# seanbonjean/llm-sharding

Measured on AMD Instinct MI355X. Metric: output_tokens_per_sec_whole_node, higher is better.
Workload: dtype bf16; 1 GPU; model=Llama-2-7B, global_batch=512, seq_len=303, parallelism=pp1, microbatches=1, batch_per_microbatch=512, prompt_len=128, concurrent_streams=1, max_seq=320

## Files before the change

csrc/build.py:

```python
#!/usr/bin/env python3
from __future__ import annotations

import argparse
import concurrent.futures as cf
import glob
import os
import shutil
import subprocess
import sys

ROOT = os.path.dirname(os.path.dirname(os.path.abspath(__file__)))
CSRC = os.path.join(ROOT, "csrc")
OUT = os.path.join(ROOT, "llm_sharding_amd", "_native")
OBJ = os.path.join(ROOT, "build", "obj")
ROCM = os.environ.get("ROCM_PATH", "/opt/rocm")


def _hipcc() -> str:
    p = os.path.join(ROCM, "bin", "hipcc")
    return p if os.path.exists(p) else (shutil.which("hipcc") or "hipcc")


def _newest_header() -> float:
    hs = glob.glob(os.path.join(CSRC, "**", "*.h"), recursive=True)
    return max((os.path.getmtime(h) for h in hs), default=0.0)


def _stale(src: str, obj: str, hdr_mtime: float) -> bool:
    if not os.path.exists(obj):
        return True
    t = os.path.getmtime(obj)
    return t < os.path.getmtime(src) or t < hdr_mtime


def _run(cmd: list) -> None:
    r = subprocess.run(cmd, stdout=subprocess.PIPE, stderr=subprocess.STDOUT, text=True)
    if r.returncode != 0:
        raise RuntimeError(f"build failed: {' '.join(cmd)}\n{r.stdout}")
    if r.stdout.strip():
        sys.stderr.write(r.stdout)


def build(force: bool = False, jobs: int = 8, arch: str = "gfx950", verbose: bool = True) -> dict:
    os.makedirs(OUT, exist_ok=True)
    os.makedirs(OBJ, exist_ok=True)
    hdr = _newest_header()
    hipcc = _hipcc()
    kernel_srcs = sorted(glob.glob(os.path.join(CSRC, "kernels", "*.hip")) +
                         glob.glob(os.path.join(CSRC, "sampling", "*.hip")) +
                         glob.glob(os.path.join(CSRC, "cache", "*.hip")) +
                         glob.glob(os.path.join(CSRC, "spec", "*.hip")) +
                         glob.glob(os.path.join(CSRC, "quant", "*.hip")))
    comm_srcs = sorted(glob.glob(os.path.join(CSRC, "comm", "*.cpp")))
    hip_flags = ["-O3", "-std=c++17", "-fPIC", f"--offload-arch={arch}", "-Wall",
                 "-Wno-unused-function", "-munsafe-fp-atomics", "-fno-slp-vectorize"]
    stamp = os.path.join(OBJ, "hip_flags.txt")
    if (open(stamp).read() if os.path.exists(stamp) else "") != " ".join(hip_flags):
        force = True
    jobs_list = []
    kobjs = []
    for s in kernel_srcs:
        o = os.path.join(OBJ, os.path.basename(s) + ".o")
        kobjs.append(o)
        if force or _stale(s, o, hdr):
            jobs_list.append([hipcc, *hip_flags, "-c", s, "-o", o])
    cobjs = []
    cxx = shutil.which("g++") or "g++"
    for s in comm_srcs:
        o = os.path.join(OBJ, os.path.basename(s) + ".o")
        cobjs.append(o)
        if force or _stale(s, o, hdr):
            jobs_list.append([cxx, "-O2", "-std=c++17", "-fPIC", "-Wall", "-c", s, "-o", o])
    if verbose and jobs_list:
        print(f"[build] compiling {len(jobs_list)} translation unit(s) for {arch}", file=sys.stderr)
    with cf.ThreadPoolExecutor(max(1, jobs)) as ex:
        list(ex.map(_run, jobs_list))
    out = {}
    klib = os.path.join(OUT, "liblsa_kernels.so")
    manifest = os.path.join(OBJ, "liblsa_kernels.objs")
    listed = open(manifest).read() if os.path.exists(manifest) else ""
    if kobjs and (force or not os.path.exists(klib) or listed != "\n".join(kobjs) or
                  os.path.getmtime(klib) < max(os.path.getmtime(o) for o in kobjs)):
        _run([hipcc, "-shared", "-fPIC", f"--offload-arch={arch}", *kobjs, "-o", klib])
        with open(manifest, "w") as f:
            f.write("\n".join(kobjs))
    with open(stamp, "w") as f:
        f.write(" ".join(hip_flags))
    audit_stamp = os.path.join(OBJ, "isa_audit.ok")
    if not os.path.exists(audit_stamp) or os.path.getmtime(audit_stamp) < os.path.getmtime(klib):
        sys.path.insert(0, CSRC)
        from isa_audit import audit
        res = audit(klib, arch)
        if res["code_objects"] == 0:
            raise RuntimeError(f"ISA audit of {klib}: no {arch} code object found in the library's offload bundle")
        if res["findings"]:
            raise RuntimeError(f"ISA audit of {klib}: back-to-back hazards {res['by_rule']}, e.g. "
                               f"{res['findings'][:3]} (csrc/isa_audit.py)")
        with open(audit_stamp, "w") as f:
            f.write(f"{res['code_objects']} code objects, {res['packed_fp32_instructions']} packed FP32 (explicit "
                    f"vector code), 0 findings under rules {sorted(res['by_rule'])}\n")
    out["kernels"] = klib
    clib = os.path.join(OUT, "liblsa_comm.so")
    if cobjs and (force or not os.path.exists(clib) or
                  os.path.getmtime(clib) < max(os.path.getmtime(o) for o in cobjs)):
        _run([cxx, "-shared", "-fPIC", *cobjs, "-o", clib, "-lpthread"])
    out["comm"] = clib
    return out


def main() -> None:
    ap = argparse.ArgumentParser()
    ap.add_argument("--force", action="store_true")
    ap.add_argument("-j", "--jobs", type=int, default=min(8, os.cpu_count() or 4))
    ap.add_argument("--arch", default=os.environ.get("PYTORCH_ROCM_ARCH", "gfx950"))
    a = ap.parse_args()
    res = build(a.force, a.jobs, a.arch)
    for k, v in res.items():
        print(f"{k}: {v}")


if __name__ == "__main__":
    main()
```

llm_sharding_amd/runtime/engine_int4.py:

```python
from __future__ import annotations

from typing import Optional

import torch

from ..ops import int4, packing
from .engine import StageEngine

PROJ = ("qkv", "o", "gate_up", "down")


class Int4StageEngine(StageEngine):
    def __init__(self, cfg, start: int, end: int, device="cpu", dtype=torch.bfloat16, *, weight_dtype: str = "int4",
                 **kw):
        if weight_dtype != "int4":
            raise ValueError(f"Int4StageEngine holds int4 weights, got weight_dtype={weight_dtype!r}")
        self.int4 = torch.device(device).type == "cuda"
        if self.int4:
            for name, (n, k) in zip(PROJ, self.proj_shapes(cfg)):
                if k % int4.INT4_GROUP:
                    raise ValueError(f"weight_dtype='int4' needs K % {int4.INT4_GROUP} == 0: the {name} projection "
                                     f"has K={k}")
        super().__init__(cfg, start, end, device, dtype, weight_dtype="bf16", **kw)

    def _prepare_layer(self, lw: dict):
        out = super()._prepare_layer(lw)
        if not self.int4:
            return out
        for name in PROJ:
            q, sc = int4.quantize_int4_groups(packing.unpack_b(getattr(out, name)))
            setattr(out, name, int4.pack_b_int4(q))
            setattr(out, name + "_s", int4.pack_scales_int4(sc))
        return out

    def _alloc_runtime(self) -> None:
        super()._alloc_runtime()
        if self.int4:
            shapes = self.proj_shapes(self.cfg)
            self.w_scratch = torch.empty(max(n * k for n, k in shapes), dtype=torch.bfloat16, device=self.device)

    def _forward_hip(self, h, slot, pos, kv_len, rows, nsplit: Optional[int] = None, tiles=None) -> torch.Tensor:
        from ..ops import hip
        cfg = self.cfg
        H, I, eps = cfg.hidden_size, cfg.intermediate_size, cfg.rms_norm_eps
        nh, nkv, hd = cfg.num_attention_heads, cfg.num_key_value_heads, cfg.head_dim
        if rows > self.max_prefill_rows and rows > self.DECODE_MAX_ROWS:
            raise ValueError(f"{rows} rows exceed max_prefill_rows={self.max_prefill_rows}")
        if h.dtype != torch.bfloat16 or not h.is_contiguous():
            h = h.to(torch.bfloat16).contiguous()
        hbuf = self.buf_h[:rows]
        if h.data_ptr() != hbuf.data_ptr():
            hbuf.copy_(h)
        decode = rows <= self.DECODE_MAX_ROWS
        if nsplit is None and tiles is None:
            kv_max = self.max_seq if decode else (int(pos.max().item()) + 1 if kv_len is None else int(kv_len.max().item()))
            nsplit = self._attn_nsplit(rows, kv_max)
        q, attn_o, act, xn = self.buf_q[:rows], self.buf_attn[:rows], self.buf_act[:rows], self.buf_xn[:rows]
        ws = self.coop_ws
        native_fp8 = False
        native_int4 = rows <= int4.INT4_MAX_ROWS
        if cfg.is_gpt2:
            return self._forward_hip_gpt2(hbuf, slot, pos, kv_len, rows, nsplit, tiles, decode, native_int4)
        wbf = self._weights_bf16

        def dec(x, w, s, N, K, epi, ep, norm=False):
            if native_int4:
                int4.gemv_int4(x, w, s, rows, N, K, epi, ep, norm=norm, eps=eps)
            else:
                hip.gemv(x, wbf(w, s, N, K), rows, N, K, epi, ep, norm=norm, eps=eps, ws=ws)

        def dec_resid(x, w, s, N, K, ep):
            pc = None if (native_fp8 or s is not None or cfg.is_gpt2 or N not in (2048, 4096, 6144, 8192)) \
                else packing.partial_config(N // 16, rows, k=K)
            if pc is None or ws.slab.numel() < pc[3] * rows * N:
                dec(x, w, s, N, K, hip.EPI_RESID, ep)
                return
            part = ws.slab[:pc[3] * rows * N].view(pc[3], rows, N)
            hip.gemv(x, w, rows, N, K, hip.EPI_PARTIAL, hip.make_epi(out=part, ldo=N), coop=pc, ws=ws,
                     out_numel=part.numel())
            hip.resid_rmsnorm_partials(hbuf, part, pc[3], rows, eps)

        def pre(x, w, s, N, K, epi, ep):
            hip.gemm(x, wbf(w, s, N, K), rows, N, K, epi, ep, ws=ws, sk_ws=self.sk_ws)

        proj_gemm = (not decode) or (rows > self.GEMV_MAX_ROWS and not native_fp8 and self.sk_ws is not None)
        part_ok = proj_gemm and self.part_k is not None and rows <= self.part_k.shape[1]

        def resid_proj(x, w, s, N, K, ep):
            pp = hip.gemm_sk_partial_plan(rows, N, K) if part_ok else None
            if pp is None:
                pre(x, w, s, N, K, hip.EPI_RESID, ep)
                return 0
            bn, sp = pp
            hip.gemm_sk(x, wbf(w, s, N, K), rows, N, K, hip.EPI_PARTIAL, hip.make_epi(out=self.part_k, ldo=N),
                        bn=bn, grid=hip.N_CU, dp=0, split=sp, ws=self.sk_ws, out_numel=self.part_k.numel())
            return sp

        fuse = proj_gemm and self.ss_buf is not None and rows <= self.ss_buf.shape[0]
        ss = self.ss_buf[:rows] if fuse else None
        ao = (self.ATTN_OPROJ and rows == 1 and tiles is None and nsplit == 1 and not proj_gemm and not native_fp8
              and self.ao_sync is not None)
        ss_valid = False
        pending = 0
        for li, lw in enumerate(self.layers):
            kc, vc = self.k_cache[li], self.v_cache[li]
            ep_qkv = hip.make_epi(out=q, k_cache=kc, v_cache=vc, slot=slot, pos=pos, cos=self.cos, sin=self.sin,
                                  ldo=q.stride(0), n_heads=nh, n_kv=nkv, head_dim=hd, t_max=self.max_seq)
            if not proj_gemm:
                dec(hbuf, lw.qkv, lw.qkv_s, cfg.qkv_size, H, hip.EPI_QKV, ep_qkv, norm=True)
            else:
                if pending and not fuse:
                    hip.resid_rmsnorm_partials(hbuf, self.part_k, pending, rows, eps, out=xn)
                    pending = 0
                    pre(xn, lw.qkv, lw.qkv_s, cfg.qkv_size, H, hip.EPI_QKV, ep_qkv)
                elif fuse:
                    if pending:
                        hip.resid_rmsnorm_partials(hbuf, self.part_k, pending, rows, eps)
                        pending = 0
                    if not ss_valid:
                        hip.row_ss(hbuf, rows, ss)
                    ep_qkv = hip.make_epi(out=q, k_cache=kc, v_cache=vc, slot=slot, pos=pos, cos=self.cos,
                                          sin=self.sin, ldo=q.stride(0), n_heads=nh, n_kv=nkv, head_dim=hd,
                                          t_max=self.max_seq, ss_in=ss, ss_eps=eps)
                    pre(hbuf, lw.qkv, lw.qkv_s, cfg.qkv_size, H, hip.EPI_QKV, ep_qkv)
                else:
                    hip.rmsnorm(hbuf, None, xn, rows, eps, H)
                    pre(xn, lw.qkv, lw.qkv_s, cfg.qkv_size, H, hip.EPI_QKV, ep_qkv)
            ep_o = hip.make_epi(out=hbuf, resid=hbuf, ldo=hbuf.stride(0), ldr=hbuf.stride(0))
            fused_o = ao and lw.o_s is None and hip.attn_oproj(q, kc, vc, slot, pos, nh, nkv, hd, attn_o, lw.o, H, ep_o,
                                                               self.ao_sync, kv_len=kv_len)
            if tiles is not None:
                hip.attn_prefill(q, kc, vc, tiles[1], nh, nkv, hd, attn_o, causal=kv_len is None, tiles_host=tiles[0])
            elif not fused_o:
                hip.attn(q, kc, vc, slot, pos, rows, nh, nkv, hd, nsplit, self.part_o, self.part_lse, attn_o,
                         kv_len=kv_len, counters=self.attn_cnt, min_chunk=self.ATTN_MIN_CHUNK)
            ep_gu = hip.make_epi(out=act, ldo=act.stride(0))
            if not proj_gemm:
                if not fused_o:
                    dec_resid(attn_o, lw.o, lw.o_s, H, cfg.q_size, ep_o)
                dec(hbuf, lw.gate_up, lw.gate_up_s, 2 * I, H, hip.EPI_SWIGLU, ep_gu, norm=True)
                dec_resid(act, lw.down, lw.down_s, H, I, ep_o)
            else:
                ep_r = hip.make_epi(out=hbuf, resid=hbuf, ldo=hbuf.stride(0), ldr=hbuf.stride(0), ss_out=ss) \
                    if fuse else ep_o
                sp = resid_proj(attn_o, lw.o, lw.o_s, H, cfg.q_size, ep_r)
                if sp:
                    hip.resid_rmsnorm_partials(hbuf, self.part_k, sp, rows, eps, out=xn)
                    pre(xn, lw.gate_up, lw.gate_up_s, 2 * I, H, hip.EPI_SWIGLU, ep_gu)
                elif fuse:
                    pre(hbuf, lw.gate_up, lw.gate_up_s, 2 * I, H, hip.EPI_SWIGLU,
                        hip.make_epi(out=act, ldo=act.stride(0), ss_in=ss, ss_eps=eps))
                else:
                    hip.rmsnorm(hbuf, None, xn, rows, eps, H)
                    pre(xn, lw.gate_up, lw.gate_up_s, 2 * I, H, hip.EPI_SWIGLU, ep_gu)
                pending = resid_proj(act, lw.down, lw.down_s, H, I, ep_r)
                ss_valid = fuse and not pending
        if pending:
            hip.resid_rmsnorm_partials(hbuf, self.part_k, pending, rows, eps)
        return hbuf

    def _weights_bf16(self, w, s, N, K):
        return w if s is None else int4.dequant_int4_packed(w, s, self.w_scratch, N, K)

    def _forward_hip_gpt2(self, hbuf, slot, pos, kv_len, rows, nsplit, tiles, decode, native_int4) -> torch.Tensor:
        from ..ops import hip
        cfg = self.cfg
        H, I, eps = cfg.hidden_size, cfg.intermediate_size, cfg.rms_norm_eps
        nh, nkv, hd = cfg.num_attention_heads, cfg.num_key_value_heads, cfg.head_dim
        q, attn_o, act, xn = self.buf_q[:rows], self.buf_attn[:rows], self.buf_act[:rows], self.buf_xn[:rows]
        ws = self.coop_ws

        def proj(x, w, s, N, K, epi, ep):
            if decode and native_int4:
                int4.gemv_int4(x, w, s, rows, N, K, epi, ep)
                return
            wb = self._weights_bf16(w, s, N, K)
            if decode:
                hip.gemv(x, wb, rows, N, K, epi, ep, ws=ws)
            else:
                hip.gemm(x, wb, rows, N, K, epi, ep, ws=ws, sk_ws=self.sk_ws)

        for li, lw in enumerate(self.layers):
            kc, vc = self.k_cache[li], self.v_cache[li]
            pe = self.pos_emb if (li == 0 and self.start == 0) else None
            hip.layernorm(hbuf, xn, lw.ln_in, lw.ln_in_b, rows, eps, pos_emb=pe, pos=pos)
            ep_qkv = hip.make_epi(out=q, k_cache=kc, v_cache=vc, slot=slot, pos=pos, ldo=q.stride(0), n_heads=nh,
                                  n_kv=nkv, head_dim=hd, t_max=self.max_seq, bias=lw.qkv_b)
            proj(xn, lw.qkv, lw.qkv_s, cfg.qkv_size, H, hip.EPI_QKV, ep_qkv)
            if tiles is not None:
                hip.attn_prefill(q, kc, vc, tiles[1], nh, nkv, hd, attn_o, causal=kv_len is None, tiles_host=tiles[0])
            else:
                hip.attn(q, kc, vc, slot, pos, rows, nh, nkv, hd, nsplit, self.part_o, self.part_lse, attn_o,
                         kv_len=kv_len, counters=self.attn_cnt, min_chunk=self.ATTN_MIN_CHUNK)
            proj(attn_o, lw.o, lw.o_s, H, cfg.q_size, hip.EPI_RESID,
                 hip.make_epi(out=hbuf, resid=hbuf, ldo=hbuf.stride(0), ldr=hbuf.stride(0), bias=lw.o_b))
            hip.layernorm(hbuf, xn, lw.ln_post, lw.ln_post_b, rows, eps)
            proj(xn, lw.gate_up, lw.gate_up_s, I, H, hip.EPI_STORE,
                 hip.make_epi(out=act, ldo=act.stride(0), bias=lw.gate_up_b, act=hip.ACT_GELU))
            proj(act, lw.down, lw.down_s, H, I, hip.EPI_RESID,
                 hip.make_epi(out=hbuf, resid=hbuf, ldo=hbuf.stride(0), ldr=hbuf.stride(0), bias=lw.down_b))
        return hbuf


def make_stage_engine(cfg, start: int, end: int, device="cpu", dtype=torch.bfloat16, *, weight_dtype: str = "bf16",
                      kv_dtype: str = "bf16", **kw) -> StageEngine:
    from .engine_kv8 import Fp8KVStageEngine, check_kv_dtype
    check_kv_dtype(kv_dtype, weight_dtype)
    if kv_dtype == "fp8" and torch.device(device).type == "cuda":
        return Fp8KVStageEngine(cfg, start, end, device, dtype, weight_dtype=weight_dtype, **kw)
    if weight_dtype == "int4":
        return Int4StageEngine(cfg, start, end, device, dtype, **kw)
    return StageEngine(cfg, start, end, device, dtype, weight_dtype=weight_dtype, **kw)
```

llm_sharding_amd/utils/runtime_config.py:

```python
from __future__ import annotations

import argparse
import dataclasses
import json
from dataclasses import dataclass, fields
from typing import Optional

import torch

BACKENDS = ("tcp", "rccl", "local")


KNOBS = {
    "LSA_LOG_LEVEL": ("env", "product", "INFO", "log level of utils/log.py"),
    "LSA_LOG_JSON": ("env", "product", "", "1 = JSON log lines"),
    "LSA_TRACE": ("env", "product", "", "directory for per-rank Chrome-trace timelines (bench --trace, serve)"),
    "LSA_DIST_TIMEOUT_S": ("env", "product", "300", "torch.distributed collective timeout of the pipeline"),
    "LSA_STARTUP_TIMEOUT_S": ("env", "product", "180", "RCCL bring-up watchdog (exit PREFLIGHT_EXIT when exceeded)"),
    "LSA_PREFLIGHT_TIMEOUT_S": ("env", "product", "30", "per-edge receive timeout of the ring preflight"),
    "LSA_IPC_TIMEOUT_S": ("env", "product", "30", "bounded spin of an IPC-ring hand-off before it poisons"),
    "LSA_IPC_ALLOC": ("env", "product", "uncached", "IPC ring buffer kind: uncached | fine (coarse is refused across GPUs)"),
    "LSA_PP_STREAMS": ("env", "product", "1", "pipeline: concurrent micro-batch streams per stage"),
    "LSA_GRAPH_COMM": ("env", "product", "1", "capture IPC-ring hand-offs inside the decode hipGraph"),
    "LSA_BENCH_ROLE": ("env", "product", "", "set by bench.py's supervisor for its worker process"),
    "LSA_BENCH_FALLBACK": ("env", "product", "", "set by bench.py when it restarted on --transport ipc"),
    "LSA_PARENT_PID": ("env", "product", "", "set by bench.py for its children (PR_SET_PDEATHSIG check)"),
    "LSA_KERNELS_SO": ("env", "diagnostic", "_native/liblsa_kernels.so", "load another build of the kernel library"),
    "LSA_GEMV_MAX_ROWS": ("env", "diagnostic", "128 (64 for MID_GEMM_SHAPES)",
                          "rows up to which decode projections stay on the GEMVs (profiles/r5_gemv_max_rows_ab.md)"),
    "LSA_GEMM_WR": ("env", "diagnostic", "1", "0 = no gemm_wr routes (profiles/r4_gemm_wr_engine_ab.txt)"),
    "LSA_ATTN_MIN_CHUNK": ("env", "diagnostic", "256", "shortest split-KV chunk in keys"),
    "LSA_ATTN_MFMA": ("env", "diagnostic", "1", "0 = no MFMA GQA decode kernel"),
    "LSA_ATTN_MFMA_MIN_ITEMS": ("env", "diagnostic", "512", "rows x kv-heads from which GQA decode uses MFMA"),
    "LSA_ATTN_GQA_NW": ("env", "diagnostic", "0", "waves of the GQA decode kernel (0 = planner)"),
    "LSA_ATTN_SMALL_MAX_WGS": ("env", "diagnostic", "", "grid size limit of the small-grid decode attention"),
    "LSA_ATTN_OPROJ": ("env", "diagnostic", "0", "1 = batch-1 attention + o projection in one launch (profiles/r6_attn_oproj.md)"),
    "LSA_AO_ABLATE": ("define", "diagnostic", "0", "attn_oproj ablation builds (scripts/probes/build_attn_oproj_ab.sh)"),
    "LSA_PREFLIGHT_FAULT": ("env", "diagnostic", "", "fault injection: 'a->b' drops the preflight message of edge a->b"),
    "LSA_SK_ABLATE": ("define", "diagnostic", "0", "gemm_sk ablation builds (scripts/sk_ablate.py)"),
    "LSA_COOP_ABLATE": ("define", "diagnostic", "0", "coop GEMV ablation builds"),
    "LSA_GEMM_SK_TUNING": ("env", "diagnostic", "", "path of a gemm_sk tuning table to use instead of ops/gemm_sk_tuning.json (A/B runs)"),
    "LSA_GEMV_TUNING": ("env", "diagnostic", "", "path of a decode-GEMV tuning table to use instead of ops/gemv_tuning.json (A/B runs)"),
    "LSA_STREAM_ABLATE": ("define", "diagnostic", "0", "gemv_stream probe ablation builds (scripts/probes/build_gemv_stream.sh)"),
    "LSA_GEMM_STAMPS": ("define", "diagnostic", "", "gemm_sk per-phase s_memrealtime stamps"),
    "LSA_COOP_STAMPS": ("define", "diagnostic", "", "coop GEMV per-phase stamps"),
    "LSA_RECORD_FULL_DEPTH": ("env", "test", "", "1 = record tests/fixtures/full_depth_7b.json instead of checking it"),
    "LSA_FULL_DEPTH_FIXTURE": ("env", "test", "tests/fixtures/full_depth_7b.json", "where the full-depth fixture lives"),
    "LSA_VARIANT_SLP": ("env", "diagnostic", "", "scripts/probes/build_kernels_variant.sh: build with SLP on"),
}


def knobs_in_effect() -> dict:
    import os
    return {k: os.environ[k] for k, v in KNOBS.items() if v[0] == "env" and k in os.environ}


@dataclass
class RuntimeConfig:
    model: str = "llama2-7b"
    shards: str = ""
    device: str = ""
    dtype: str = "bfloat16"
    backend: str = "rccl"
    batch: int = 32
    microbatches: int = 0
    streams: int = 1
    max_seq: int = 2048
    prefill_budget: int = 2048
    max_new_tokens: int = 128
    use_graph: bool = True
    causal: bool = True
    port: int = 40700
    seed: int = 0
    trace_dir: str = ""
    log_level: str = "INFO"

    def __post_init__(self):
        if self.backend not in BACKENDS:
            raise ValueError(f"backend must be one of {BACKENDS}, got {self.backend!r}")
        if self.batch < 0 or self.max_seq < 2 or self.prefill_budget < 1:
            raise ValueError("batch must be >= 0 (0 = auto), max_seq and prefill_budget positive")

    @classmethod
    def add_arguments(cls, ap: argparse.ArgumentParser) -> argparse.ArgumentParser:
        for f in fields(cls):
            flag = "--" + f.name.replace("_", "-")
            if f.type in (bool, "bool"):
                if f.default:
                    ap.add_argument("--no-" + f.name.replace("_", "-"), dest=f.name, action="store_false",
                                    help=f"disable {f.name}")
                else:
                    ap.add_argument(flag, dest=f.name, action="store_true")
            else:
                typ = int if f.type in (int, "int") else str
                ap.add_argument(flag, dest=f.name, type=typ, default=f.default)
        return ap

    @classmethod
    def from_args(cls, ns: argparse.Namespace) -> "RuntimeConfig":
        return cls(**{f.name: getattr(ns, f.name) for f in fields(cls) if hasattr(ns, f.name)})

    def to_json(self) -> str:
        return json.dumps(dataclasses.asdict(self))

    @classmethod
    def from_json(cls, s: str) -> "RuntimeConfig":
        d = json.loads(s)
        return cls(**{k: v for k, v in d.items() if k in {f.name for f in fields(cls)}})

    def torch_device(self, local_rank: int = 0) -> torch.device:
        if self.device:
            return torch.device(self.device)
        return torch.device("cuda", local_rank) if torch.cuda.is_available() else torch.device("cpu")

    def torch_dtype(self, device: Optional[torch.device] = None) -> torch.dtype:
        if device is not None and device.type == "cuda":
            return torch.bfloat16
        return getattr(torch, self.dtype)

    def model_and_source(self):
        from ..config import LlamaConfig, get_preset
        from ..runtime.engine import RandomSource, ShardFolderSource
        if self.shards:
            cfg = LlamaConfig.from_pretrained(self.shards)
            return cfg, ShardFolderSource(self.shards, cfg)
        cfg = get_preset(self.model)
        return cfg, RandomSource(cfg, self.seed)


__all__ = ["RuntimeConfig", "BACKENDS"]
```

Baseline: 31010 tokens/s.

## Add split-K GEMM with distributed band fixup for residual projections

Measured after the change: 31360 tokens/s (median of 6 runs). 1.01x the previous value.

```diff
diff --git a/csrc/build.py b/csrc/build.py
--- a/csrc/build.py
+++ b/csrc/build.py
@@ -47,6 +47,7 @@
     hdr = _newest_header()
     hipcc = _hipcc()
     kernel_srcs = sorted(glob.glob(os.path.join(CSRC, "kernels", "*.hip")) +
+                         glob.glob(os.path.join(CSRC, "gemm_skp", "*.hip")) +
                          glob.glob(os.path.join(CSRC, "sampling", "*.hip")) +
                          glob.glob(os.path.join(CSRC, "cache", "*.hip")) +
                          glob.glob(os.path.join(CSRC, "spec", "*.hip")) +
diff --git a/csrc/gemm_skp/gemm_skp.hip b/csrc/gemm_skp/gemm_skp.hip
--- /dev/null
+++ b/csrc/gemm_skp/gemm_skp.hip
@@ -0,0 +1,278 @@
+
+#define lsa_gemm_sk lsa_gemm_skp_unused_decl_(); template <int SKP_UNUSED_> int lsa_gemm_skp_unused_
+#define lsa_gemm_sk_set_stamps lsa_gemm_skp_set_stamps
+#define g_stamps g_stamps_skp
+#include "../kernels/gemm_sk.hip"
+#undef lsa_gemm_sk
+
+namespace {
+
+constexpr int SKP_MAX_C = 8;
+
+LSA_DEVICE void vm_wait_rows(int rows) {
+  switch (rows) {
+    case 0: vm_wait<0>(); break;
+    case 1: vm_wait<4>(); break;
+    case 2: vm_wait<8>(); break;
+    case 3: vm_wait<12>(); break;
+    case 4: vm_wait<16>(); break;
+    case 5: vm_wait<20>(); break;
+    case 6: vm_wait<24>(); break;
+    default: vm_wait<28>(); break;
+  }
+}
+
+LSA_DEVICE void ticket_issue(unsigned& old, unsigned* counter) {
+  asm volatile("global_atomic_add %0, %1, %2, off sc0" : "+v"(old) : "v"(counter), "v"(1u) : "memory");
+}
+LSA_DEVICE void ticket_wait(unsigned& old) { asm volatile("s_waitcnt vmcnt(0)" : "+v"(old)::"memory"); }
+
+template <int BM, int BN, int EPI, int NB>
+struct Band {
+  using K_ = Kern<BM, BN, EPI, NB>;
+  using G_ = Geo<BM, BN, NB>;
+  static constexpr int FM = K_::FM, FN = K_::FN, TM = K_::TM, TN = K_::TN;
+  static_assert(FN == 4 && TN == 64 && FM <= 8, "a fragment row is one wave's 16 rows x 64 columns");
+  static_assert(EPI == EPI_STORE || EPI == EPI_RESID, "band epilogues");
+
+  LSA_DEVICE static int blk_off(const K_& k, int i, int j) { return ((k.w * FM * FN + i * FN + j) * 64 + k.lane) * 16; }
+
+  LSA_DEVICE static __amdgpu_buffer_rsrc_t slab_rsrc(float* slab, int unit) {
+    return __builtin_amdgcn_make_buffer_rsrc(slab + (size_t)unit * 2 * (size_t)(BM * BN), (short)0, BM * BN * 4,
+                                             0x00020000);
+  }
+
+  static constexpr int CH = (BM == 256 && BN == 256) ? 2 : 4;
+  template <typename UnitOf>
+  LSA_DEVICE static void reduce_row(const K_& k, float* slab, int C, int c, UnitOf unit_of, int i,
+                                    const f32x4_t (&own)[FN], f32x4_t (&t)[FN]) {
+#pragma unroll
+    for (int ch = 0; ch < SKP_MAX_C / CH; ++ch) {
+      if (ch * CH >= C) break;
+      f32x4_t ld[CH][FN];
+#pragma unroll
+      for (int q = 0; q < CH; ++q) {
+        const int ci = ch * CH + q;
+        if (ci < C && ci != c) {
+          const __amdgpu_buffer_rsrc_t sr = slab_rsrc(slab, unit_of(ci));
+#pragma unroll
+          for (int j = 0; j < FN; ++j)
+            ld[q][j] = __builtin_bit_cast(f32x4_t, __builtin_amdgcn_raw_buffer_load_b128(sr, blk_off(k, i, j), 0, 16 ));
+        } else {
+#pragma unroll
+          for (int j = 0; j < FN; ++j) ld[q][j] = own[j];
+        }
+      }
+#pragma unroll
+      for (int q = 0; q < CH; ++q) {
+        const int ci = ch * CH + q;
+        if (ci < C) {
+#pragma unroll
+          for (int j = 0; j < FN; ++j) {
+            if (ch == 0 && q == 0) t[j] = ld[q][j]; else t[j] += ld[q][j];
+          }
+        }
+      }
+    }
+  }
+
+  LSA_DEVICE static void epilogue_row(const K_& k, const EpiArgs& ep, const f32x4_t (&t)[FN], int mt, int nt, int i) {
+    const SkParams& P = *k.p;
+    constexpr int ELD = G_::ELD;
+    float* img = reinterpret_cast<float*>(k.smem) + k.w * (G_::EROWS * ELD);
+    const int lane = k.lane;
+#pragma unroll
+    for (int j = 0; j < FN; ++j)
+#pragma unroll
+      for (int r = 0; r < 4; ++r) img[(4 * (lane >> 4) + r) * ELD + j * 16 + (lane & 15)] = t[j][r];
+    __builtin_amdgcn_fence(__ATOMIC_RELEASE, "wavefront");
+    __builtin_amdgcn_wave_barrier();
+    __builtin_amdgcn_fence(__ATOMIC_ACQUIRE, "wavefront");
+    const int row = lane / FN, j = lane % FN;
+    const int m = mt * BM + k.wr * TM + i * 16 + row;
+    const int col_base = nt * BN + k.wc * TN;
+    const int c0 = col_base + j * 16;
+    const float* src = img + row * ELD + j * 16;
+    float v[16];
+#pragma unroll
+    for (int q = 0; q < 4; ++q) *reinterpret_cast<f32x4_t*>(v + 4 * q) = *reinterpret_cast<const f32x4_t*>(src + 4 * q);
+    if (EPI == EPI_RESID && ep.ss_out) {
+      float ssq = 0.f;
+      if (m < P.M) {
+        epi_bias16(ep, c0, v);
+        const bf16_raw* rr = ep.resid + (size_t)m * ep.ldr + c0;
+        float x0[8], x1[8];
+        unpack8(ld16(rr), x0);
+        unpack8(ld16(rr + 8), x1);
+#pragma unroll
+        for (int q = 0; q < 8; ++q) {
+          x0[q] += v[q];
+          x1[q] += v[q + 8];
+        }
+        const u32x4_t p0 = pack8(x0), p1 = pack8(x1);
+        bf16_raw* o = ep.out + (size_t)m * ep.ldo + c0;
+        st16(o, p0);
+        st16(o + 8, p1);
+        unpack8(p0, x0);
+        unpack8(p1, x1);
+        ssq = ss16(x0, x1);
+      }
+#pragma unroll
+      for (int o = 1; o < FN; o <<= 1) ssq = __fadd_rn(ssq, __shfl_xor(ssq, o, 64));
+      if (m < P.M && (lane % FN) == 0) ep.ss_out[(size_t)m * ep.ss_n + (col_base >> 6)] = ssq;
+    } else if (m < P.M) {
+      epi_row16<EPI>(ep, m, c0, v);
+    }
+    __builtin_amdgcn_fence(__ATOMIC_RELEASE, "wavefront");
+    __builtin_amdgcn_wave_barrier();
+    __builtin_amdgcn_fence(__ATOMIC_ACQUIRE, "wavefront");
+  }
+};
+
+template <int BM, int BN, int EPI, int NB>
+__global__ __launch_bounds__(NTHR) void gemm_skp_kernel(const bf16_raw* __restrict__ A, const bf16_raw* __restrict__ W,
+                                                         SkParams prm, EpiArgs ep, float* __restrict__ slab,
+                                                         unsigned* __restrict__ counters, int tile_major) {
+  using K_ = Kern<BM, BN, EPI, NB>;
+  using B_ = Band<BM, BN, EPI, NB>;
+  constexpr int FM = K_::FM, FN = K_::FN;
+  __shared__ __attribute__((aligned(16))) unsigned char smem[Geo<BM, BN, NB>::SMEM];
+  K_ k;
+  k.smem = smem;
+  k.A = A;
+  k.W = W;
+  k.p = &prm;
+  k.tid = threadIdx.x;
+  k.lane = threadIdx.x & 63;
+  k.w = __builtin_amdgcn_readfirstlane(threadIdx.x >> 6);
+  k.wr = k.w / K_::WN;
+  k.wc = k.w % K_::WN;
+  k.group = k.w >> 2;
+  const int C = prm.split, tiles = prm.sk_tiles, U = prm.G;
+  const int hw = blockIdx.x;
+  int su;
+  {
+    const int q = U / 8, r = U % 8, x = hw % 8;
+    su = (x < r ? x * (q + 1) : r * (q + 1) + (x - r) * q) + hw / 8;
+  }
+  const int ts = tile_major ? su / C : su % tiles;
+  const int c = tile_major ? su % C : su / tiles;
+  auto unit_of = [&](int ci) { return tile_major ? ts * C + ci : ts + ci * tiles; };
+  const int ka = c * prm.NKT / C, kb = (c + 1) * prm.NKT / C;
+  int mt, nt;
+  tile_coords(prm, ts, mt, nt);
+  f32x4_t acc[FM][FN];
+#pragma unroll
+  for (int i = 0; i < FM; ++i)
+#pragma unroll
+    for (int j = 0; j < FN; ++j) acc[i][j] = f32x4_t{0.f, 0.f, 0.f, 0.f};
+  k.run_segment(acc, mt, nt, ka, kb);
+  LSA_STAMP(2);
+
+  int band[FM];
+#pragma unroll
+  for (int i = 0; i < FM; ++i) band[i] = (k.w + i) % C;
+
+  const __amdgpu_buffer_rsrc_t own = B_::slab_rsrc(slab, su);
+  for (int s = 0; s < C; ++s) {
+    const int b = c + s < C ? c + s : c + s - C;
+#pragma unroll
+    for (int i = 0; i < FM; ++i)
+      if (band[i] == b) {
+#pragma unroll
+        for (int j = 0; j < FN; ++j)
+          __builtin_amdgcn_raw_buffer_store_b128(__builtin_bit_cast(u32x4_t, acc[i][j]), own, B_::blk_off(k, i, j), 0, 16);
+      }
+  }
+  unsigned* cnt = counters + (size_t)ts * SKP_MAX_C;
+  unsigned old = 0u;
+  int rem = FM;
+  for (int s = 0; s < C; ++s) {
+    const int b = c + s < C ? c + s : c + s - C;
+#pragma unroll
+    for (int i = 0; i < FM; ++i) rem -= band[i] == b ? 1 : 0;
+    vm_wait_rows(rem);
+    barrier();
+    if (k.w == s && k.lane == 0) ticket_issue(old, &cnt[b]);
+  }
+  ticket_wait(old);
+  unsigned char* last = smem + Geo<BM, BN, NB>::SMEM - 16;
+  if (k.w < C && k.lane == 0) last[k.w] = old == (unsigned)(C - 1);
+  __syncthreads();
+  LSA_STAMP(3);
+
+  for (int s = 0; s < C; ++s) {
+    if (!__builtin_amdgcn_readfirstlane((int)last[s])) continue;
+    const int b = c + s < C ? c + s : c + s - C;
+#pragma unroll
+    for (int i = 0; i < FM; ++i)
+      if (band[i] == b) {
+        f32x4_t t[FN];
+        B_::reduce_row(k, slab, C, c, unit_of, i, acc[i], t);
+        B_::epilogue_row(k, ep, t, mt, nt, i);
+      }
+    if (k.tid == 0) __hip_atomic_store(&cnt[b], 0u, __ATOMIC_RELAXED, __HIP_MEMORY_SCOPE_AGENT);
+  }
+  LSA_STAMP(5);
+}
+
+template <int BM, int BN, int EPI, int NB>
+int launch_p(const bf16_raw* A, const bf16_raw* W, const SkParams& prm, const EpiArgs& ep, float* slab, unsigned* cnt,
+             int tile_major, hipStream_t s) {
+  gemm_skp_kernel<BM, BN, EPI, NB><<<prm.G, NTHR, 0, s>>>(A, W, prm, ep, slab, cnt, tile_major);
+  LSA_CHECK_LAUNCH();
+  return LSA_OK;
+}
+
+template <int BM, int EPI>
+int dispatch_p(const bf16_raw* A, const bf16_raw* W, const SkParams& prm, const EpiArgs& ep, float* slab, unsigned* cnt,
+               int bn, int nb, int tile_major, hipStream_t s) {
+  if (bn == 256) {
+    if constexpr (BM == 128) {
+      if (nb == 3) return launch_p<BM, 256, EPI, 3>(A, W, prm, ep, slab, cnt, tile_major, s);
+    }
+    return launch_p<BM, 256, EPI, 2>(A, W, prm, ep, slab, cnt, tile_major, s);
+  }
+  return nb == 3 ? launch_p<BM, 128, EPI, 3>(A, W, prm, ep, slab, cnt, tile_major, s)
+                 : launch_p<BM, 128, EPI, 2>(A, W, prm, ep, slab, cnt, tile_major, s);
+}
+
+}
+
+extern "C" int lsa_gemm_skp(const void* a, int lda, const void* wp, int M, int N, int K, int epi, const EpiArgs* ep,
+                            int bm, int bn, int nb, int contributors, int tile_major, int group_m, float* slab,
+                            unsigned* counters, long long slab_floats, int n_counters, hipStream_t stream) {
+  if (M < 1 || K < BK || K % BK || lda < K || lda % 8 || !ep) return LSA_BAD_SHAPE;
+  if (bn != 256 && bn != 128) return LSA_UNSUPPORTED;
+  if (bm != 256 && bm != 128) return LSA_UNSUPPORTED;
+  if (epi != EPI_STORE && epi != EPI_RESID) return LSA_UNSUPPORTED;
+  if (nb == 0) nb = (bn == 128 || (bm == 128 && bn == 256)) ? 3 : 2;
+  if (nb != 2 && !(nb == 3 && (bn == 128 || (bm == 128 && bn == 256)))) return LSA_UNSUPPORTED;
+  if (N < bn || N % bn || group_m < 1 || (tile_major != 0 && tile_major != 1)) return LSA_BAD_SHAPE;
+  if (contributors < 2 || contributors > SKP_MAX_C || contributors > K / BK) return LSA_BAD_SHAPE;
+  if (!ep->out || (epi == EPI_RESID && !ep->resid)) return LSA_BAD_SHAPE;
+  if (ep->ss_in || (ep->ss_out && (epi != EPI_RESID || N % 64 || ep->ss_n != N / 64))) return LSA_BAD_SHAPE;
+  SkParams prm;
+  prm.M = M;
+  prm.N = N;
+  prm.K = K;
+  prm.lda = lda;
+  prm.MT = (M + bm - 1) / bm;
+  prm.NT = N / bn;
+  prm.NKT = K / BK;
+  prm.group_m = group_m;
+  const long long tiles = (long long)prm.MT * prm.NT;
+  if (tiles * contributors > 1024) return LSA_BAD_SHAPE;
+  prm.G = (int)tiles * contributors;
+  prm.dp_rounds = 0;
+  prm.sk_tiles = (int)tiles;
+  prm.split = contributors;
+  if (!slab || !counters || slab_floats < 2LL * prm.G * bm * bn || n_counters < prm.sk_tiles * SKP_MAX_C)
+    return LSA_BAD_SHAPE;
+  const bf16_raw* A = static_cast<const bf16_raw*>(a);
+  const bf16_raw* W = static_cast<const bf16_raw*>(wp);
+#define LSA_GP(E) (bm == 256 ? dispatch_p<256, E>(A, W, prm, *ep, slab, counters, bn, nb, tile_major, stream) \
+                     : dispatch_p<128, E>(A, W, prm, *ep, slab, counters, bn, nb, tile_major, stream))
+  return epi == EPI_STORE ? LSA_GP(EPI_STORE) : LSA_GP(EPI_RESID);
+#undef LSA_GP
+}
diff --git a/llm_sharding_amd/ops/gemm_skp.py b/llm_sharding_amd/ops/gemm_skp.py
--- /dev/null
+++ b/llm_sharding_amd/ops/gemm_skp.py
@@ -0,0 +1,134 @@
+from __future__ import annotations
+
+import ctypes
+import functools
+import os
+from typing import Optional
+
+import torch
+
+from . import hip
+
+MAX_CONTRIBUTORS = 8
+MAX_GRID = 1024
+TUNING_FILE = os.environ.get("LSA_GEMM_SKP_TUNING") or os.path.join(os.path.dirname(os.path.abspath(__file__)),
+                                                                   "skp_tuning.txt")
+
+
+def enabled() -> bool:
+    return os.environ.get("LSA_GEMM_SKP", "1") != "0"
+
+
+def tiles(M: int, N: int, bm: int, bn: int) -> int:
+    return -(-M // bm) * (N // bn)
+
+
+def check_plan(M: int, N: int, K: int, bm: int, bn: int, contributors: int) -> Optional[str]:
+    if bm not in (128, 256) or bn not in (128, 256):
+        return f"tile {bm}x{bn}: bm and bn are 128 or 256"
+    if M < 1 or K < 64 or K % 64 or N < bn or N % bn:
+        return f"shape M={M} N={N} K={K} does not tile by {bm}x{bn}x64"
+    if not 2 <= contributors <= MAX_CONTRIBUTORS:
+        return f"{contributors} contributors: 2..{MAX_CONTRIBUTORS}"
+    if contributors > K // 64:
+        return f"{contributors} contributors for {K // 64} K-tiles"
+    if tiles(M, N, bm, bn) * contributors > MAX_GRID:
+        return f"{tiles(M, N, bm, bn)} tiles x {contributors} contributors exceed {MAX_GRID} workgroups"
+    return None
+
+
+def slab_floats(M: int, N: int, bm: int, bn: int, contributors: int) -> int:
+    return 2 * tiles(M, N, bm, bn) * contributors * bm * bn
+
+
+def n_counters(M: int, N: int, bm: int, bn: int) -> int:
+    return tiles(M, N, bm, bn) * MAX_CONTRIBUTORS
+
+
+class SkpWorkspace:
+
+    def __init__(self, device, slab_floats: int, counters: int):
+        self.slab = torch.empty(slab_floats, dtype=torch.float32, device=device)
+        self.counters = torch.zeros(counters, dtype=torch.int32, device=device)
+
+    @classmethod
+    def for_plan(cls, device, M: int, N: int, bm: int, bn: int, contributors: int) -> "SkpWorkspace":
+        return cls(device, slab_floats(M, N, bm, bn, contributors), n_counters(M, N, bm, bn))
+
+
+def parse_table(text: str) -> dict:
+    out: dict = {}
+    for ln, line in enumerate(text.splitlines(), 1):
+        line = line.split("#", 1)[0].strip()
+        if not line:
+            continue
+        f = line.split()
+        if len(f) != 7:
+            raise ValueError(f"skp tuning table line {ln}: 7 integers expected, got {line!r}")
+        M, N, K, bm, bn, C, tm = (int(v) for v in f)
+        why = check_plan(M, N, K, bm, bn, C)
+        if why or tm not in (0, 1):
+            raise ValueError(f"skp tuning table line {ln}: {why or 'tile_major is 0 or 1'}")
+        out.setdefault((N, K), []).append((M, (bm, bn, C, tm)))
+    return out
+
+
+@functools.lru_cache(maxsize=1)
+def _table() -> dict:
+    if not os.path.exists(TUNING_FILE):
+        return {}
+    with open(TUNING_FILE) as f:
+        return parse_table(f.read())
+
+
+def lookup(table: dict, M: int, N: int, K: int) -> Optional[tuple]:
+    m128 = -(-M // 128)
+    cands = [(abs(m - M), cfg) for m, cfg in table.get((N, K), ()) if -(-m // 128) == m128]
+    if not cands:
+        return None
+    cfg = min(cands)[1]
+    return None if check_plan(M, N, K, cfg[0], cfg[1], cfg[2]) else cfg
+
+
+def plan(M: int, N: int, K: int) -> Optional[tuple]:
+    if not enabled():
+        return None
+    return lookup(_table(), M, N, K)
+
+
+_BOUND = False
+
+
+def _lib():
+    global _BOUND
+    L = hip.lib()
+    if not _BOUND:
+        if not hasattr(L, "lsa_gemm_skp"):
+            raise RuntimeError("liblsa_kernels.so has no lsa_gemm_skp: rebuild (python csrc/build.py)")
+        vp, i = ctypes.c_void_p, ctypes.c_int
+        L.lsa_gemm_skp.argtypes = [vp, i, vp, i, i, i, i, ctypes.POINTER(hip.EpiArgs), i, i, i, i, i, i, vp, vp,
+                                   ctypes.c_longlong, i, vp]
+        L.lsa_gemm_skp.restype = i
+        _BOUND = True
+    return L
+
+
+def gemm_skp(a: torch.Tensor, wp: torch.Tensor, M: int, N: int, K: int, epi: int, ep, *, bm: int, bn: int,
+             contributors: int, tile_major: int = 0, nb: int = 0, group_m: int = 8, ws=None) -> None:
+    hip._req(hip._is_bf16_cuda(a, wp), "gemm_skp: bf16 cuda tensors required")
+    hip._req(wp.numel() == N * K and K % 64 == 0 and K >= 64, "gemm_skp: packed weight shape")
+    hip._req(a.dim() == 2 and a.shape[0] >= M >= 1 and a.shape[1] >= K and a.stride(1) == 1 and a.stride(0) % 8 == 0
+             and a.data_ptr() % 16 == 0, "gemm_skp: A must be [>=M, >=K] row-major with 16-B aligned rows")
+    hip._req(epi in (hip.EPI_STORE, hip.EPI_RESID), "gemm_skp: EPI_STORE / EPI_RESID")
+    hip._check_epi(epi, ep, N)
+    why = check_plan(M, N, K, bm, bn, contributors)
+    hip._req(why is None, f"gemm_skp: {why}")
+    hip._req(tile_major in (0, 1) and nb in (0, 2, 3), "gemm_skp: tile_major 0 / 1, nb 0 / 2 / 3")
+    if ws is None:
+        ws = hip.default_sk_workspace(a.device)
+    hip._req(ws.slab.numel() >= slab_floats(M, N, bm, bn, contributors) and
+             ws.counters.numel() >= n_counters(M, N, bm, bn), f"gemm_skp: workspace too small for {bm}x{bn} x {contributors}")
+    rc = _lib().lsa_gemm_skp(hip._p(a), a.stride(0), hip._p(wp), M, N, K, epi, ctypes.byref(ep), bm, bn, nb, contributors,
+                             tile_major, group_m, hip._p(ws.slab), hip._p(ws.counters), ws.slab.numel(),
+                             ws.counters.numel(), hip._stream())
+    hip._check(rc, "lsa_gemm_skp")
diff --git a/llm_sharding_amd/runtime/engine_int4.py b/llm_sharding_amd/runtime/engine_int4.py
--- a/llm_sharding_amd/runtime/engine_int4.py
+++ b/llm_sharding_amd/runtime/engine_int4.py
@@ -210,4 +210,7 @@
         return Fp8KVStageEngine(cfg, start, end, device, dtype, weight_dtype=weight_dtype, **kw)
     if weight_dtype == "int4":
         return Int4StageEngine(cfg, start, end, device, dtype, **kw)
+    if torch.device(device).type == "cuda":
+        from .engine_skp import SkpStageEngine
+        return SkpStageEngine(cfg, start, end, device, dtype, weight_dtype=weight_dtype, **kw)
     return StageEngine(cfg, start, end, device, dtype, weight_dtype=weight_dtype, **kw)
diff --git a/llm_sharding_amd/runtime/engine_skp.py b/llm_sharding_amd/runtime/engine_skp.py
--- /dev/null
+++ b/llm_sharding_amd/runtime/engine_skp.py
@@ -0,0 +1,82 @@
+from __future__ import annotations
+
+from typing import Optional
+
+import torch
+
+from ..ops import gemm_skp
+from .engine import StageEngine
+
+SKP_MIN_ROWS, SKP_MAX_ROWS = 385, 512
+
+
+class SkpStageEngine(StageEngine):
+
+    def skp_plans(self, rows: int, tiles=None) -> Optional[tuple]:
+        from ..ops import hip
+        cfg = self.cfg
+        if not (SKP_MIN_ROWS <= rows <= SKP_MAX_ROWS) or tiles is not None or cfg.is_gpt2 or self.fp8:
+            return None
+        if not gemm_skp.enabled() or self.device.type != "cuda" or self.sk_ws is None:
+            return None
+        if rows <= self.GEMV_MAX_ROWS or self.ss_buf is None or rows > self.ss_buf.shape[0]:
+            return None
+        H, I = cfg.hidden_size, cfg.intermediate_size
+        shapes = ((H, cfg.q_size), (H, I))
+        if self.part_k is not None and rows <= self.part_k.shape[1] and \
+                any(hip.gemm_sk_partial_plan(rows, N, K) is not None for N, K in shapes):
+            return None
+        plans = tuple(gemm_skp.plan(rows, N, K) for N, K in shapes)
+        for (N, K), p in zip(shapes, plans):
+            if p is not None and (self.sk_ws.slab.numel() < gemm_skp.slab_floats(rows, N, p[0], p[1], p[2]) or
+                                  self.sk_ws.counters.numel() < gemm_skp.n_counters(rows, N, p[0], p[1])):
+                return None
+        return plans if any(p is not None for p in plans) else None
+
+    def _forward_hip(self, h, slot, pos, kv_len, rows, nsplit: Optional[int] = None, tiles=None) -> torch.Tensor:
+        plans = self.skp_plans(rows, tiles)
+        if plans is None:
+            return super()._forward_hip(h, slot, pos, kv_len, rows, nsplit, tiles)
+        from ..ops import hip
+        cfg = self.cfg
+        H, I, eps = cfg.hidden_size, cfg.intermediate_size, cfg.rms_norm_eps
+        nh, nkv, hd = cfg.num_attention_heads, cfg.num_key_value_heads, cfg.head_dim
+        if rows > self.max_prefill_rows and rows > self.DECODE_MAX_ROWS:
+            raise ValueError(f"{rows} rows exceed max_prefill_rows={self.max_prefill_rows}")
+        if h.dtype != torch.bfloat16 or not h.is_contiguous():
+            h = h.to(torch.bfloat16).contiguous()
+        hbuf = self.buf_h[:rows]
+        if h.data_ptr() != hbuf.data_ptr():
+            hbuf.copy_(h)
+        if nsplit is None:
+            kv_max = int(pos.max().item()) + 1 if kv_len is None else int(kv_len.max().item())
+            nsplit = self._attn_nsplit(rows, kv_max)
+        q, attn_o, act = self.buf_q[:rows], self.buf_attn[:rows], self.buf_act[:rows]
+        ws, sk_ws = self.coop_ws, self.sk_ws
+        ss = self.ss_buf[:rows]
+
+        def resid_proj(x, w, N, K, ep, p):
+            if p is None:
+                hip.gemm(x, w, rows, N, K, hip.EPI_RESID, ep, ws=ws, sk_ws=sk_ws)
+            else:
+                gemm_skp.gemm_skp(x, w, rows, N, K, hip.EPI_RESID, ep, bm=p[0], bn=p[1], contributors=p[2],
+                                  tile_major=p[3], ws=sk_ws)
+
+        ss_valid = False
+        for li, lw in enumerate(self.layers):
+            kc, vc = self.k_cache[li], self.v_cache[li]
+            if not ss_valid:
+                hip.row_ss(hbuf, rows, ss)
+            ep_qkv = hip.make_epi(out=q, k_cache=kc, v_cache=vc, slot=slot, pos=pos, cos=self.cos, sin=self.sin,
+                                  ldo=q.stride(0), n_heads=nh, n_kv=nkv, head_dim=hd, t_max=self.max_seq,
+                                  ss_in=ss, ss_eps=eps)
+            hip.gemm(hbuf, lw.qkv, rows, cfg.qkv_size, H, hip.EPI_QKV, ep_qkv, ws=ws, sk_ws=sk_ws)
+            hip.attn(q, kc, vc, slot, pos, rows, nh, nkv, hd, nsplit, self.part_o, self.part_lse, attn_o,
+                     kv_len=kv_len, counters=self.attn_cnt, min_chunk=self.ATTN_MIN_CHUNK)
+            ep_r = hip.make_epi(out=hbuf, resid=hbuf, ldo=hbuf.stride(0), ldr=hbuf.stride(0), ss_out=ss)
+            resid_proj(attn_o, lw.o, H, cfg.q_size, ep_r, plans[0])
+            hip.gemm(hbuf, lw.gate_up, rows, 2 * I, H, hip.EPI_SWIGLU,
+                     hip.make_epi(out=act, ldo=act.stride(0), ss_in=ss, ss_eps=eps), ws=ws, sk_ws=sk_ws)
+            resid_proj(act, lw.down, H, I, ep_r, plans[1])
+            ss_valid = True
+        return hbuf
diff --git a/llm_sharding_amd/utils/runtime_config.py b/llm_sharding_amd/utils/runtime_config.py
--- a/llm_sharding_amd/utils/runtime_config.py
+++ b/llm_sharding_amd/utils/runtime_config.py
@@ -29,6 +29,9 @@
     "LSA_GEMV_MAX_ROWS": ("env", "diagnostic", "128 (64 for MID_GEMM_SHAPES)",
                           "rows up to which decode projections stay on the GEMVs (profiles/r5_gemv_max_rows_ab.md)"),
     "LSA_GEMM_WR": ("env", "diagnostic", "1", "0 = no gemm_wr routes (profiles/r4_gemm_wr_engine_ab.txt)"),
+    "LSA_GEMM_SKP": ("env", "diagnostic", "1", "0 = no gemm_skp routes: the residual projections keep gemm_sk "
+                     "(profiles/skp_fixup.md)"),
+    "LSA_GEMM_SKP_TUNING": ("env", "diagnostic", "", "path of another gemm_skp tuning table (ops/skp_tuning.txt)"),
     "LSA_ATTN_MIN_CHUNK": ("env", "diagnostic", "256", "shortest split-KV chunk in keys"),
     "LSA_ATTN_MFMA": ("env", "diagnostic", "1", "0 = no MFMA GQA decode kernel"),
     "LSA_ATTN_MFMA_MIN_ITEMS": ("env", "diagnostic", "512", "rows x kv-heads from which GQA decode uses MFMA"),
```
